# AgentCooper2002/AudioDiffuser

Hardware: AMD Instinct MI355X
Metric: audio samples/sec (16384-sample waveform, 50-step Heun) (higher is better)
Workload: dtype bf16; 1 GPU; BASELINE configs[1]: UNet1d 64 ch (c2), 16384-sample waveforms, KarrasSchedule N=50 heun, batch 64/GPU, random-init weights; global_batch=64, sampler=heun, num_steps=50, nfe=99, hipgraph=True, parallelism=batch-sharded x1, one all-gather

## Files before the change

### audiodiffuser_amd/csrc/adf_gemm.h

```cpp
#pragma once
#include "adf_common.h"

namespace adf {

constexpr int kARows = 144;
constexpr int kTapGroup = 3;

struct GemmSeg {
    const void* src0;
    const void* src1;
    int c0, c1;
    const float* ab;
    GnFinalizeArgs gn;
    float scale1;
    int act;
    int taps, stride, off0, step;
    const void* w;
    const void* wfrag;
    int nchunk;
};

struct GemmArgs {
    GemmSeg seg[2];
    int nseg;
    int B, lin, mrows, n, n_pad;
    int gn_ready;
    int flat;
    int seg_rows;
    const float* bias0;
    const float* bias1;
    int bias_mod;
    const void* res;
    int gelu;
    void* out;
    int out_rows, out_c;
    int scatter_f, scatter_pad;
    int phase_c;
    double* stats;
    int stats_groups;
};

template <int N>
__device__ __forceinline__ void gemm_bias_load(const GemmArgs& a, const int (&bi)[N], const bool (&ok)[N], float (&out)[N]) {
    const bool h0 = a.bias0 != nullptr, h1 = a.bias1 != nullptr;
    const float* const dmy = (const float*)a.seg[0].w;
    const float* const p0 = h0 ? a.bias0 : dmy;
    const float* const p1 = h1 ? a.bias1 : dmy;
    float v0[N], v1[N];
#pragma unroll
    for (int k = 0; k < N; ++k) {
        const int idx = ok[k] ? bi[k] : 0;
        v0[k] = p0[h0 ? idx : 0]; v1[k] = p1[h1 ? idx : 0];
// ... 1215 lines not shown
```

### audiodiffuser_amd/csrc/adf_gemm.hip

```cpp
#include "adf_gemm.h"
#include "adf_gemm_pp.h"
#include "adf_gemm_rb.h"
#include "adf_gemm_rbx3.h"
#include "adf_gemm_up.h"
#include "adf_kernels.h"
#include <cstdio>
#include <cstdlib>
#include <cstring>
#include <vector>


#ifdef ADF_RB_STAMP
namespace adf { __device__ unsigned long long adf_rb_stamps[8 * 16]; }
extern "C" int adf_debug_rb_stamps(unsigned long long* out) {
    return (int)hipMemcpyFromSymbol(out, HIP_SYMBOL(adf::adf_rb_stamps), sizeof(unsigned long long) * 8 * 16);
}
#endif

#ifdef ADF_RB_TL
namespace adf { __device__ unsigned adf_rb_tl[2 * 8 * 128]; }
extern "C" int adf_debug_rb_timeline(unsigned* out) {
    return (int)hipMemcpyFromSymbol(out, HIP_SYMBOL(adf::adf_rb_tl), sizeof(unsigned) * 2 * 8 * 128);
}
#endif
// ... 153 lines not shown
            e.src = (const char*)(from1 ? s1 : s0) + (size_t)(from1 ? c - c0 : c) * f.esz;
            e.pitch = (unsigned)(from1 ? c1 : c0) * (unsigned)f.esz;
            e.w = (const char*)w + (size_t)(c / f.blk_ch) * taps * a.n_pad * kRowBytes;
            e.tab = table ? c * 8 : -1;
            e.scale = from1 ? scale1 : 1.0f;
        }
    };
    add_seg(g0.src0, g0.src1, g0.c0, g0.c1, g0.w, 3, !raw0, 1.0f);
    r.h.nb3 = nb;
    if (a.nseg > 1) {
        const GemmSeg& g1 = a.seg[1];
        if (g1.taps != 1 || g1.off0 != 0 || g1.stride != 1 || g1.step != 1 || g1.ab || g1.gn.gamma || g1.act) return false;
        if (!seg_ok(g1.c0, g1.c1, nb)) return false;
        add_seg(g1.src0, g1.src1, g1.c0, g1.c1, g1.w, 1, false, g1.scale1);
    }
    r.h.res = a.nseg == 1 ? a.res : nullptr;
    r.h.nb1 = nb - r.h.nb3;
    r.h.B = a.B; r.h.L = a.mrows;
    r.h.n = a.n;
    r.h.gn = g0.gn;
    r.h.bias0 = a.bias0; r.h.bias1 = a.bias1;
    r.h.out = a.out;
    r.h.stats = nullptr; r.h.stats_groups = 0;
    if (a.phase_c && (!raw0 || (a.phase_c & (a.phase_c - 1)) || a.phase_c < 64 || a.n % a.phase_c)) return false;
    if (a.stats) {
        const int sc = a.phase_c ? a.phase_c : a.out_c;
        const int gs = a.stats_groups > 0 ? sc / a.stats_groups : 0;
        if (!(gs > 0 && gs * a.stats_groups == sc && (gs & (gs - 1)) == 0 && gs >= 8 && gs <= 64)) return false;
        r.h.stats = a.stats; r.h.stats_groups = a.stats_groups;
        r.h.stats_mod = a.phase_c;
    }
    return true;
}
static int rb_num_cus() {
    static int num_cu_dev[kMaxDevices] = {};
    int& n = num_cu_dev[current_device()];
    if (n == 0 && (hipDeviceGetAttribute(&n, hipDeviceAttributeMultiprocessorCount, current_device()) != hipSuccess || n < 1)) n = 256;
    return n;
}

bool try_launch_rb(const GemmArgs& a, const void* ident, long long min_tiles, hipStream_t stream, const char** err, bool dry = false) {
    *err = nullptr;
    (void)ident;
    auto pow2 = [](int v) { return v > 0 && (v & (v - 1)) == 0; };
    RbArgs r;
    bool raw0 = false;
    if (!rb_build_args(a, RbForm{2, 64, kRbMaxBlk, true}, r, raw0)) return false;
    static long long m128_nh = -1;
    if (m128_nh < 0) m128_nh = adf_tuning("ADF_RB_M128_NH", 1);
    auto shape = [&](int tm_, int& nh_) -> long long {
        if (a.mrows % tm_ || !pow2(a.mrows / tm_)) return 0;
        const long long tiles_m = (long long)a.B * (a.mrows / tm_);
        nh_ = (a.n == 256 && tiles_m >= min_tiles) ? 2 : 1;
        return tiles_m * (a.n / (kPpTN * nh_));
    };
    int tm = 256, nh = 1;
    long long tiles_total = shape(256, nh);
    bool wide128 = false;
    if (tiles_total < min_tiles) {
        tm = 128;
        tiles_total = shape(128, nh);
        if (m128_nh == 2 && a.n == 256 && nh == 1 && tiles_total >= min_tiles) { nh = 2; tiles_total /= 2; wide128 = true; }
    }
    if (tiles_total > (1 << 22) || tiles_total < (wide128 ? min_tiles / 2 : min_tiles)) return false;
    r.h.tiles_n = a.n / (kPpTN * nh);
    r.h.tm_shift = 0;
    while ((1 << r.h.tm_shift) < a.mrows / tm) ++r.h.tm_shift;
    r.h.tiles_total = (int)tiles_total;
    if (dry) return true;
    static bool attr_done[kMaxDevices] = {};
    const int dev = current_device();
    if (!attr_done[dev]) {
        bool ok = true;
        for (const void* k : {(const void*)conv_gemm_rb_kernel<1, false, 2>, (const void*)conv_gemm_rb_kernel<2, false, 2>, (const void*)conv_gemm_rb_kernel<1, true, 2>,
                              (const void*)conv_gemm_rb_kernel<2, true, 2>, (const void*)conv_gemm_rb_kernel<1, false, 1>, (const void*)conv_gemm_rb_kernel<2, false, 1>,
                              (const void*)conv_gemm_rb_kernel<1, true, 1>, (const void*)conv_gemm_rb_kernel<2, true, 1>})
            ok = ok && hipFuncSetAttribute(k, hipFuncAttributeMaxDynamicSharedMemorySize, kRbLds) == hipSuccess;
        if (!ok) {
            *err = "hipFuncSetAttribute(MaxDynamicSharedMemorySize, rb) failed";
            return true;
        }
        attr_done[dev] = true;
    }
    const int ncu = rb_num_cus();
    const long long grid = tiles_total < ncu ? tiles_total : ncu;
    auto go = [&](auto kern) { hipLaunchKernelGGL(kern, dim3((unsigned)grid), dim3(512), kRbLds, stream, r); };
    if (tm == 256) {
        if (nh == 2 && raw0) go(conv_gemm_rb_kernel<2, true, 2>);
        else if (nh == 2) go(conv_gemm_rb_kernel<2, false, 2>);
        else if (raw0) go(conv_gemm_rb_kernel<1, true, 2>);
        else go(conv_gemm_rb_kernel<1, false, 2>);
    } else {
        if (nh == 2 && raw0) go(conv_gemm_rb_kernel<2, true, 1>);
        else if (nh == 2) go(conv_gemm_rb_kernel<2, false, 1>);
        else if (raw0) go(conv_gemm_rb_kernel<1, true, 1>);
        else go(conv_gemm_rb_kernel<1, false, 1>);
    }
    if (hipGetLastError() != hipSuccess) *err = "conv_gemm_rb: launch failed";
    return true;
}

bool try_launch_rbx3(const GemmArgs& a, long long min_tiles, hipStream_t stream, const char** err, bool dry = false) {
// ... 76 lines not shown
    constexpr int lds = 4 * ks_wave_lds(MT, NT);
    constexpr int TM = 32 * MT, TN = 32 * NT;
    static bool attr_done[kMaxDevices] = {};
    bool& attr_set = attr_done[current_device()];
    auto kern = conv_gemm_ksplit_kernel<T, MT, NT>;
    if (!attr_set) {
        if (hipFuncSetAttribute((const void*)kern, hipFuncAttributeMaxDynamicSharedMemorySize, lds) != hipSuccess)
            return "hipFuncSetAttribute(MaxDynamicSharedMemorySize, ksplit) failed";
        attr_set = true;
    }
    const int tiles_n = (a.n_pad + TN - 1) / TN;
    const long long tiles_m = a.flat ? ((long long)a.B * a.mrows + TM - 1) / TM : (long long)((a.mrows + TM - 1) / TM) * a.B;
    const long long blocks = tiles_m * tiles_n;
    if (blocks <= 0 || blocks > 0x7fffffffLL) return "conv_gemm_ksplit: bad grid";
    hipLaunchKernelGGL(kern, dim3((unsigned)blocks), dim3(256), lds, stream, a);
    return hipGetLastError() == hipSuccess ? nullptr : "conv_gemm_ksplit: launch failed";
}

template <typename T>
const char* dispatch(const GemmArgs& a, int tm, int tn, hipStream_t s) {
    if (tm == 128 && tn == 128) return launch_variant<T, 2, 2, 2, 2>(a, s);
    if (tm == 128 && tn == 64) return launch_variant<T, 2, 1, 2, 2>(a, s);
    if (tm == 128 && tn == 32) return launch_variant<T, 1, 1, 4, 1>(a, s);
    if (tm == 64 && tn == 128) return launch_variant<T, 1, 2, 2, 2>(a, s);
    if (tm == 64 && tn == 64) return launch_variant<T, 1, 1, 2, 2>(a, s);
    if (tm == 64 && tn == 32) return launch_variant<T, 1, 1, 2, 1>(a, s);
    if (tm == 32 && tn == 128) return launch_variant<T, 1, 1, 1, 4>(a, s);
    if (tm == 32 && tn == 64) return launch_variant<T, 1, 1, 1, 2>(a, s);
    return launch_variant<T, 1, 1, 1, 1>(a, s);
}

}

static void trace_route(const char* route, const GemmArgs& a, int tm, int tn) {
    static int on = -1;
    if (on < 0) on = adf_route_switch("ADF_GEMM_TRACE", 0);
    if (!on) return;
    fprintf(stderr, "[adf gemm] %-6s B=%d lin=%d mrows=%d n=%d/%d nseg=%d seg0(c=%d+%d taps=%d stride=%d off0=%d step=%d ab=%d act=%d)", route, a.B, a.lin, a.mrows,
            a.n, a.n_pad, a.nseg, a.seg[0].c0, a.seg[0].c1, a.seg[0].taps, a.seg[0].stride, a.seg[0].off0, a.seg[0].step, a.seg[0].ab != nullptr, a.seg[0].act);
    if (a.nseg > 1) fprintf(stderr, " seg1(c=%d+%d taps=%d ab=%d)", a.seg[1].c0, a.seg[1].c1, a.seg[1].taps, a.seg[1].ab != nullptr);
    fprintf(stderr, " res=%d gelu=%d scatter=%d out=%dx%d stats=%d flat=%d tile=%dx%d\n", a.res != nullptr, a.gelu, a.scatter_f, a.out_rows, a.out_c, a.stats != nullptr,
            a.flat, tm, tn);
}

static long long rb_min_tiles() {
    static int use_rb = -1;
    if (use_rb < 0) use_rb = adf_route_switch("ADF_GEMM_RB", 1);
    return use_rb == 0 ? -1 : (use_rb >= 2 ? 32 : 256);
}
static long long rbx3_min_tiles() {
    static int use_rbx3 = -1;
    if (use_rbx3 < 0) use_rbx3 = adf_route_switch("ADF_GEMM_RBX3", 1);
    return use_rbx3 == 0 ? -1 : (use_rbx3 >= 2 ? 32 : 256);
}
bool conv_gemm_phase_eligible(const GemmArgs& a, int dtype) {
    const long long mt = dtype == 2 ? rbx3_min_tiles() : rb_min_tiles();
    if (dtype == 0 || mt < 0 || !a.phase_c || a.flat) return false;
    const char* err = nullptr;
    return dtype == 2 ? try_launch_rbx3(a, mt, nullptr, &err, true) : try_launch_rb(a, nullptr, mt, nullptr, &err, true);
}

const char* launch_conv_gemm(const GemmArgs& a_in, int dtype, hipStream_t stream, bool* stats_fused) {
    const bool dtype_bf16 = dtype == 1, x3 = dtype == 2;
    GemmArgs a = a_in;
    if (stats_fused) *stats_fused = false;
    if (a.phase_c) {
        const long long mt = x3 ? rbx3_min_tiles() : rb_min_tiles();
        if (dtype == 0 || mt < 0 || a.flat) return "conv_gemm: a 3-tap-form transposed conv that conv_gemm_rb_kernel does not take";
        const char* err = nullptr;
        auto go = [&]() { return x3 ? try_launch_rbx3(a, mt, stream, &err) : try_launch_rb(a, nullptr, mt, stream, &err); };
        bool taken = go();
        if (!taken && a.stats) { a.stats = nullptr; taken = go(); }
        if (!taken) return "conv_gemm: a 3-tap-form transposed conv that conv_gemm_rb_kernel does not take";
        if (stats_fused) *stats_fused = a.stats != nullptr;
        trace_route(x3 ? "rbx3" : "rb", a, 256, 128);
        return err;
    }
    if (a.nseg < 1 || a.nseg > 2) return "conv_gemm: nseg must be 1 or 2";
    if (a.n_pad % 32) return "conv_gemm: n_pad must be a multiple of 32";
    const int epc = dtype_bf16 ? 8 : 4;
    if (a.n % epc || a.out_c % epc) return "conv_gemm: output channels must be a multiple of a 16-byte chunk";
    const long long esz = dtype_bf16 ? 2 : 4;
    if ((long long)a.B * a.out_rows * a.out_c * esz >= (1LL << 32)) return "conv_gemm: output tensor must be < 4 GiB";
    const bool gn_pending = a.seg[0].gn.gamma != nullptr;
    static int gn_in_kernel = -1;
    if (gn_in_kernel < 0) gn_in_kernel = (int)adf_tuning("ADF_GEMM_GN", 1);
    auto settle_gn = [&](bool in_kernel) -> const char* {
        if (!gn_pending) return nullptr;
        const GnFinalizeArgs& gn = a.seg[0].gn;
        const int gn_gs = gn.G > 0 ? (gn.c0 + gn.c1) / gn.G : 0;
        in_kernel = in_kernel && gn_in_kernel && gn_gs > 0 && gn.c0 % gn_gs == 0;
        const char* err = nullptr;
        if (!in_kernel) {
            if (!a.gn_ready) err = launch_gn_finalize(a.seg[0].gn, stream);
            a.seg[0].gn.gamma = nullptr;
        }
        return err;
    };
    if (a.nseg > 1) a.seg[1].gn.gamma = nullptr;
    bool raw = true;
    for (int s = 0; s < a.nseg; ++s) {
        const GemmSeg& g = a.seg[s];
        if (g.c0 % epc || g.c1 % epc) return "conv_gemm: channel counts must be multiples of a 16-byte chunk";
        if (g.step != 1 && g.step != -1) return "conv_gemm: step must be +-1";
        if (g.taps < 1 || g.stride < 1) return "conv_gemm: bad taps/stride";
        if (g.ab) raw = false;
        if ((long long)a.B * a.lin * (g.c0 > g.c1 ? g.c0 : g.c1) * esz >= (1LL << 32)) return "conv_gemm: input tensor must be < 4 GiB";
    }
// ... 102 lines not shown
        }
    }
    {
        static int use_pp = -1;
        if (use_pp < 0) use_pp = adf_route_switch("ADF_GEMM_PP", 1);
        int ptm = 0;
        if (use_pp && dtype_bf16 && !flat && tm == 128) {
            const long long t256 = pp_eligible(a, 256) ? (long long)a.B * (a.mrows / 256) * (a.n_pad / kPpTN) : 0;
            const long long t128 = pp_eligible(a, 128) ? (long long)a.B * (a.mrows / 128) * (a.n_pad / kPpTN) : 0;
            const long long need = use_pp >= 2 ? 128 : 256;
            if (t256 >= need) ptm = 256;
            else if (t128 >= need && use_pp != 3) ptm = 128;
        }
        {
            static int use_rb = -1;
            if (use_rb < 0) use_rb = adf_route_switch("ADF_GEMM_RB", 1);
            const bool rb_raw = !gn_pending && !a.seg[0].ab && !a.seg[0].act && a.nseg == 1 && !a.res && a.seg[0].taps == 3;
            const long long rbx3_mt = rbx3_min_tiles();
            if (rbx3_mt >= 0 && x3 && !flat && ((gn_pending && gn_in_kernel && !a.gn_ready) || rb_raw)) {
                const char* err = nullptr;
                GemmArgs b = a;
                b.stats = a_in.stats;
                if (try_launch_rbx3(b, rbx3_mt, stream, &err)) {
                    if (stats_fused) *stats_fused = a_in.stats != nullptr;
                    trace_route("rbx3", a, 256, 128);
                    return err;
                }
            }
            if (use_rb && dtype_bf16 && !flat && ((gn_pending && gn_in_kernel && !a.gn_ready) || rb_raw)) {
                const char* err = nullptr;
                const void* ident = nullptr;
                GemmArgs b = a;
                b.stats = a_in.stats;
                if (try_launch_rb(b, ident, use_rb >= 2 ? 32 : 256, stream, &err)) {
                    if (stats_fused) *stats_fused = a_in.stats != nullptr;
                    trace_route("rb", a, 256, 128);
                    return err;
                }
            }
        }
        if (ptm) {
            static int pp_linear = -1;
            if (pp_linear < 0) pp_linear = (int)adf_tuning("ADF_GEMM_PP_LINEAR", 0);
            const bool linear = a.seg[0].taps == 1 && a.nseg == 1;
            const bool take = linear ? pp_linear != 0 : (use_pp == 2 || !a.res);
            if (take) {
                if (a_in.stats) {
                    const int gs = a.stats_groups > 0 ? a.out_c / a.stats_groups : 0;
                    const bool ok = gs > 0 && gs * a.stats_groups == a.out_c && (gs & (gs - 1)) == 0 && gs >= 8 && gs <= 64;
                    a.stats = ok ? a_in.stats : nullptr;
                    if (stats_fused) *stats_fused = ok;
                }
                if (a.res) {
                    const char* err = nullptr;
                    const void* ident = pp_identity(a.n, stream, &err);
                    if (!ident) return err;
                    GemmSeg& g = a.seg[1];
                    g = GemmSeg{};
                    g.src0 = a.res; g.src1 = nullptr; g.c0 = a.n; g.c1 = 0; g.ab = nullptr; g.scale1 = 1.0f; g.act = 0;
                    g.taps = 1; g.stride = 1; g.off0 = 0; g.step = 1; g.w = ident; g.nchunk = a.n / 64;
                    a.nseg = 2;
                    a.res = nullptr;
                }
                if (const char* e = settle_gn(a.seg[0].taps == 3)) return e;
                trace_route("pp", a, ptm, 128);
                return ptm == 256 ? launch_pp<2>(a, stream) : launch_pp<1>(a, stream);
            }
        }
    }
// ... 35 lines not shown
```

### audiodiffuser_amd/csrc/adf_gemm_rb.h

```cpp
#pragma once
#include "adf_gemm.h"
#include "adf_gemm_pp.h"
#include <type_traits>

namespace adf {

#ifdef ADF_RB_STAMP
extern __device__ unsigned long long adf_rb_stamps[8 * 16];
#endif

#ifdef ADF_RB_TL
extern __device__ unsigned adf_rb_tl[2 * 8 * 128];
constexpr int kRbLds = kPpLds + 3072;
#else
constexpr int kRbLds = kPpLds;
#endif
constexpr int kRbMaxBlk = 24;
#ifndef ADF_RB_KNOCK
#define ADF_RB_KNOCK 0
#endif
#ifndef ADF_RB_DOT2
#define ADF_RB_DOT2 1
#endif
#ifndef ADF_RB_NT
#define ADF_RB_NT 0
#endif
#ifndef ADF_RB_W3
#define ADF_RB_W3 1
#endif
#ifndef ADF_RB_PRIO
#define ADF_RB_PRIO 4
#endif
#ifndef ADF_RB_FILL2
#define ADF_RB_FILL2 1
#endif
#ifndef ADF_RB_PRESLAB
#define ADF_RB_PRESLAB 1
#endif


struct RbBlk {
    const char* src;
    const char* w;
    unsigned pitch;
    int tab;
    float scale;
    int pad_;
};

struct RbHead {
    int nb3, nb1;
    int B, L;
    int tm_shift;
    int tiles_n;
    int tiles_total;
    int n;
    GnFinalizeArgs gn;
    const float* bias0; const float* bias1;
    void* out;
    const void* res;
    double* stats; int stats_groups;
    int stats_mod;
};
struct RbArgs {
    RbHead h;
    RbBlk blk[kRbMaxBlk];
};

__device__ __forceinline__ void rb_dma2(const char* base, unsigned va, unsigned vb, unsigned la, unsigned lb) {
    asm volatile("s_mov_b32 m0, %3\n\ts_nop 0\n\tglobal_load_lds_dwordx4 %1, %0\n\t"
                 "s_mov_b32 m0, %4\n\ts_nop 0\n\tglobal_load_lds_dwordx4 %2, %0"
                 :: "s"(base), "v"(va), "v"(vb), "s"(la), "s"(lb) : "memory");
}
__device__ __forceinline__ void rb_dma1(const char* base, unsigned va, unsigned la) {
    asm volatile("s_mov_b32 m0, %2\n\ts_nop 0\n\tglobal_load_lds_dwordx4 %1, %0" :: "s"(base), "v"(va), "s"(la) : "memory");
}

template <int I, int N, typename F>
__device__ __forceinline__ void rb_static_for(F&& f) {
    if constexpr (I < N) {
        f(std::integral_constant<int, I>{});
        rb_static_for<I + 1, N>(f);
    }
}

template <int NH, bool RAW, int MH = 2>
__global__ void __launch_bounds__(512) conv_gemm_rb_kernel(const RbArgs a) {
    typedef bf16_t T;
    constexpr int TM = 128 * MH, HP = TM / 8;
    constexpr int TNB = kPpTN * NH;
    constexpr bool W3 = ADF_RB_W3 == 2 || (ADF_RB_W3 == 1 && (MH == 1 || NH == 2)) || (ADF_RB_W3 == 3 && MH == 1) || (ADF_RB_W3 == 4 && (MH == 1 || NH == 1));
    extern __shared__ __attribute__((aligned(16))) char smem[];
    const RbHead H = a.h;
    const RbBlk e_first[3] = {a.blk[0], a.blk[1], a.blk[2]};
    asm volatile("" :: "s"(H.nb3), "s"(H.tiles_total), "s"(H.gn.stats0), "s"(H.gn.gamma), "s"(H.gn.film), "s"(H.bias0), "s"(H.out), "s"(H.stats),
                 "s"(e_first[0].src), "s"(e_first[1].src), "s"(e_first[2].src), "s"(e_first[0].tab), "s"(e_first[1].tab), "s"(e_first[2].tab));
    char* const ldsScr = smem + kPpOffScr;
    char* const ldsTab = smem + kPpOffTab;
    float* const ldsBias = (float*)(smem + kPpOffBias);

    const int tid = threadIdx.x, lane = tid & 63;
    const int wave = __builtin_amdgcn_readfirstlane(tid >> 6);
    const int r = lane & 31, h = lane >> 5;
    const int wm = wave >> 1, wn = wave & 1;
    const int lrow = lane >> 3;
    const int chunk = (lane & 7) ^ ((((wave & 1) << 2) + (lane >> 4)) & 7);
    const int srow = wave * 8 + lrow;
    const unsigned lane_lds = (unsigned)lane * 16u;

    if (ADF_RB_PRIO == 4) __builtin_amdgcn_s_setprio(3);
    if (ADF_RB_PRIO == 1 && wave >= 4) __builtin_amdgcn_s_setprio(1);
    if (ADF_RB_PRIO == 3 && wave >= 4) __builtin_amdgcn_s_setprio(2);
    const int nblk_grid = (int)gridDim.x, bidx = (int)blockIdx.x;
    const int t_lo = (int)((unsigned)bidx * (unsigned)H.tiles_total / (unsigned)nblk_grid);
    const int t_hi = (int)((unsigned)(bidx + 1) * (unsigned)H.tiles_total / (unsigned)nblk_grid);
    const int ntiles = t_hi - t_lo;
    if (ntiles <= 0) return;
    const int nb3 = H.nb3, nb1 = H.nb1, nb = nb3 + nb1;
    const int ctot0 = H.gn.c0 + H.gn.c1;
    const int tn_shift = H.tiles_n > 1 ? 1 : 0;
    const int tm_mask = (1 << H.tm_shift) - 1;

    struct Tile { int b0, m0, n0; };
    auto tile_of = [&](int tseq) __attribute__((always_inline)) -> Tile {
        const int t = t_lo + tseq;
        const int tml = t >> tn_shift;
        Tile g;
        g.n0 = (t & (H.tiles_n - 1)) * TNB;
        g.b0 = tml >> H.tm_shift;
        g.m0 = (tml & tm_mask) * TM;
        return g;
    };
    const int b_first = tile_of(0).b0;

    struct Blk {
        const char* abase;
        const char* w;
        unsigned pitch;
        int tab;
        float scale;
        int edge;
        int taps;
    };
    int d_t = 0, d_k = 0;
    Tile d_tile = tile_of(0);
    auto make_desc_of = [&](const RbBlk& e) __attribute__((always_inline)) -> Blk {
        Blk d;
        const int three = d_k < nb3;
        const int p_lo = d_tile.m0 - three;
        d.pitch = e.pitch;
        d.abase = e.src + (long long)(d_tile.b0 * H.L + p_lo) * (long long)e.pitch;
        d.w = e.w + (unsigned)d_tile.n0 * (unsigned)kRowBytes;
        d.tab = e.tab >= 0 ? ((d_tile.b0 - b_first) & 1) * kPpTab + e.tab : -1;
        d.scale = e.scale;
        d.taps = three ? 3 : 1;
        d.edge = three ? ((d_tile.m0 == 0 ? 1 : 0) | (d_tile.m0 + TM >= H.L ? 2 : 0)) : 0;
        return d;
    };
    auto make_desc = [&]() __attribute__((always_inline)) -> Blk { return make_desc_of(a.blk[d_k]); };
    auto advance = [&]() __attribute__((always_inline)) {
        if (++d_k == nb) {
            d_k = 0;
            if (++d_t < ntiles) d_tile = tile_of(d_t);
        }
    };
    const unsigned slab = (unsigned)H.n * (unsigned)kRowBytes;

    const unsigned colbytes = (unsigned)chunk * 16u;
    auto issue_a01 = [&](const Blk& d, unsigned st) __attribute__((always_inline)) {
        if (ADF_RB_KNOCK & 2) return;
        const unsigned v = (unsigned)srow * d.pitch + colbytes;
        const unsigned v0 = ((d.edge & 1) && srow == 0) ? v + d.pitch : v;
        const unsigned l = st + (unsigned)wave * 1024u;
        rb_dma2(d.abase, v0, v + 64u * d.pitch, l, l + 8192u);
    };
    auto issue_a23 = [&](const Blk& d, unsigned st) __attribute__((always_inline)) {
        if ((ADF_RB_KNOCK & 2) || MH == 1) return;
        const unsigned v = (unsigned)(srow + 128) * d.pitch + colbytes;
        const unsigned l = st + (unsigned)wave * 1024u + 16384u;
        rb_dma2(d.abase, v, v + 64u * d.pitch, l, l + 8192u);
    };
    auto issue_halo = [&](const Blk& d, unsigned st) __attribute__((always_inline)) {
        if (ADF_RB_KNOCK & 2) return;
        if (wave == 0 && d.taps == 3) {
            const unsigned vh = (unsigned)TM * d.pitch + ((d.edge & 2) ? 0u : (unsigned)lrow * d.pitch) + colbytes;
            if (lane < 16) rb_dma1(d.abase, vh, st + (unsigned)HP * 1024u);
        }
    };
    const unsigned wlane = (unsigned)srow * (unsigned)kRowBytes + colbytes;
// ... 116 lines not shown
        char* const ldsH = smem + st + HP * 1024 + lane_lds;
        const bool halo = wave == 0 && d.taps == 3 && lane < 16;
        const bool act = true;
        float fa[8], fb[8];
        load_ab(d, 0, 8, fa, fb);
#pragma unroll
        for (int u = 0; u < 2 * MH; ++u) {
            const u32x4_t q = *(const u32x4_t*)(ldsA + u * 8192);
            const u32x2_t lo = silu4(u32x2_t{q.x, q.y}, fa, fb, act), hi = silu4(u32x2_t{q.z, q.w}, fa + 4, fb + 4, act);
            *(u32x4_t*)(ldsA + u * 8192) = u32x4_t{lo.x, lo.y, hi.x, hi.y};
        }
        if (halo) {
            const u32x4_t q = *(const u32x4_t*)ldsH;
            const u32x2_t lo = silu4(u32x2_t{q.x, q.y}, fa, fb, act), hi = silu4(u32x2_t{q.z, q.w}, fa + 4, fb + 4, act);
            *(u32x4_t*)ldsH = u32x4_t{lo.x, lo.y, hi.x, hi.y};
        }
        zero_fill(d, st);
    };

    f32x16_t acc[NH][MH][2];
    unsigned abase0[3];
#pragma unroll
    for (int t = 0; t < 3; ++t) {
        const int row = wm * 32 * MH + r + t, f = (row >> 1) & 7;
        abase0[t] = (unsigned)(row * kPpRow + ((h ^ (f & 1)) << 4) + ((f >> 1) << 5));
    }
    const int fw = (r >> 1) & 7;
    const unsigned wbase0 = (unsigned)((wn * 64 + r) * kPpRow + ((h ^ (fw & 1)) << 4) + ((fw >> 1) << 5));
    unsigned wadr[4];
#pragma unroll
    for (int ks = 0; ks < 4; ++ks) wadr[ks] = (unsigned)kPpOffW + (wbase0 ^ (unsigned)(ks << 5));

    unsigned ws0 = 0u, ws1 = (unsigned)kPpWStage, ws2 = 2u * (unsigned)kPpWStage;
    auto substep = [&](auto tapc, auto wstc, auto nhc, unsigned sa_, auto work, auto mid) __attribute__((always_inline)) {
        constexpr int TAP = decltype(tapc)::value;
        constexpr int WST = decltype(wstc)::value;
        constexpr int H = decltype(nhc)::value;
        const char* const pw = smem + (W3 ? ws0 : (unsigned)(WST * kPpWStage));
        unsigned aadr[4];
#pragma unroll
        for (int ks = 0; ks < 4; ++ks) aadr[ks] = sa_ + (abase0[TAP] ^ (unsigned)(ks << 5));
        bf16x8_t fa[2][MH], fb[2][2];
#pragma unroll
        for (int i = 0; i < MH; ++i) fa[0][i] = *(const bf16x8_t*)(smem + aadr[0] + i * 32 * kPpRow);
#pragma unroll
        for (int j = 0; j < 2; ++j) fb[0][j] = *(const bf16x8_t*)(pw + wadr[0] + j * 32 * kPpRow);
#pragma unroll
        for (int ks = 0; ks < 4; ++ks) {
            const int cur = ks & 1, nxt = cur ^ 1;
            if (ks + 1 < 4) {
#pragma unroll
                for (int i = 0; i < MH; ++i) fa[nxt][i] = *(const bf16x8_t*)(smem + aadr[ks + 1] + i * 32 * kPpRow);
#pragma unroll
                for (int j = 0; j < 2; ++j) fb[nxt][j] = *(const bf16x8_t*)(pw + wadr[ks + 1] + j * 32 * kPpRow);
            }
#pragma unroll
            for (int i = 0; i < MH; ++i)
#pragma unroll
                for (int j = 0; j < 2; ++j) {
                    if (!(ADF_RB_KNOCK & 8)) acc[H][i][j] = __builtin_amdgcn_mfma_f32_32x32x16_bf16(fa[cur][i], fb[cur][j], acc[H][i][j], 0, 0, 0);
                    else { asm volatile("" :: "v"(fa[cur][i]), "v"(fb[cur][j])); }
                    __builtin_amdgcn_sched_barrier(0);
                    if (!(ADF_RB_KNOCK & 1)) work(ks * 2 * MH + i * 2 + j);
                    __builtin_amdgcn_sched_barrier(0);
                }
            mid(ks);
            if (ADF_RB_PRIO == 4) {
                if (ks == 0) __builtin_amdgcn_s_setprio(2);
                else if (ks == 1) __builtin_amdgcn_s_setprio(1);
                else if (ks == 2) __builtin_amdgcn_s_setprio(0);
            }
            if (ADF_RB_PRIO == 2 && ks == 1 && wave >= 4) __builtin_amdgcn_s_setprio(2);
            if (ADF_RB_PRIO == 3 && ks == 1 && wave >= 4) __builtin_amdgcn_s_setprio(0);
            __builtin_amdgcn_sched_barrier(0);
        }
        if (ADF_RB_PRIO == 2 && wave >= 4) __builtin_amdgcn_s_setprio(0);
        if (ADF_RB_PRIO == 3 && wave >= 4) __builtin_amdgcn_s_setprio(2);
        if (ADF_RB_PRIO == 4) __builtin_amdgcn_s_setprio(3);
    };

    struct Part {
        u32x2_t raw[3];
        float ta[8], tb[8];
        float x[4], u[4];
        u32x2_t pk;
        float ec, ed;
        unsigned hraw;
        float ha, hb, hx, hu;
    };
    const unsigned halo_e = (unsigned)wave * 16u + ((unsigned)lane & 15u);
    auto half_of = [](int P, int k) constexpr -> int { return P < 2 ? P + 2 * k : 6 + k; };
    auto part_begin = [&](auto partc, const Blk& dn, unsigned sn, Part& p) __attribute__((always_inline)) {
        constexpr int P = decltype(partc)::value;
        char* const ldsN = smem + sn + wave * 1024 + lane_lds;
        if (P == 0) {
            load_ab(dn, 0, 4, p.ta, p.tb);
            p.ec = dn.tab >= 0 ? -1.4426950408889634f : 0.0f;
            p.ed = dn.tab >= 0 ? 0.0f : -200.0f;
        } else if (P == 1) load_ab(dn, 4, 4, p.ta + 4, p.tb + 4);
        constexpr int NOWN = MH == 2 ? (P < 2 ? 3 : 2) : (P < 2 ? 2 : 0);
#pragma unroll
        for (int k = 0; k < NOWN; ++k) {
            const int hh = half_of(P, k);
            p.raw[k] = *(const u32x2_t*)(ldsN + (hh >> 1) * 8192 + (hh & 1) * 8);
        }
        if (P == 2) {
            p.hraw = *(const unsigned short*)(smem + sn + HP * 1024 + halo_e * 2u);
            if (dn.tab >= 0) {
                const f32x2_t t = *(const f32x2_t*)(ldsTab + dn.tab + (halo_e & 63u) * 8u);
                p.ha = t.x; p.hb = t.y;
            } else { p.ha = dn.scale; p.hb = 0.f; }
// ... 179 lines not shown
    unsigned* const tl_lds = (unsigned*)(smem + kPpOffBias + 1024) + wave * 128;
    auto tl = [&](int id) __attribute__((always_inline)) {
        if (tl_which >= 0 && id < 128) {
            const unsigned long long t = __builtin_amdgcn_s_memtime();
            if (lane == 0) tl_lds[id] = (unsigned)t;
        }
    };
    auto tl_real = [&](int id) __attribute__((always_inline)) {
        if (tl_which >= 0) {
            const unsigned long long t = __builtin_amdgcn_s_memrealtime();
            if (lane == 0) { tl_lds[id] = (unsigned)t; tl_lds[id + 1] = (unsigned)(t >> 32); }
        }
    };
    if (tl_which >= 0) for (int i = lane; i < 128; i += 64) tl_lds[i] = 0u;
    int tl_sub = 0;
    tl_real(120);
    tl(0);
#else
    auto tl = [&](int) __attribute__((always_inline)) {};
#endif
    kstamp(11);
    tl(110);
    const bool hb0 = H.bias0 != nullptr, hb1 = H.bias1 != nullptr;
    const float* const dummy_f = (const float*)a.blk[0].w;
    const int bidx_l = tid < H.n ? tid : 0;
    const float b0v = (hb0 ? H.bias0 : dummy_f)[bidx_l], b1v = (hb1 ? H.bias1 : dummy_f)[bidx_l];
    GnLoaded gl = {};
    if constexpr (!RAW) gl = gn_load(b_first, tid < ctot0 ? tid : ctot0 - 1);
    tl(111);
    Blk dc = make_desc_of(e_first[0]);
    advance();
    issue_a01(dc, 0u); issue_a23(dc, 0u); issue_halo(dc, 0u);
    issue_w(dc.w, 0);
    if (W3 && !ADF_RB_FILL2) issue_w(dc.w + (unsigned)(1 / NH) * slab + (unsigned)(1 % NH) * (unsigned)kPpWStage, 1);
    Blk d1 = make_desc_of(e_first[1]);
    advance();
    if (!ADF_RB_FILL2) { issue_a01(d1, (unsigned)kPpAStage); issue_a23(d1, (unsigned)kPpAStage); issue_halo(d1, (unsigned)kPpAStage); }
    Blk d2 = make_desc_of(d_k == 0 ? e_first[0] : e_first[2]);
    advance();
    tl(112);
#ifdef ADF_RB_TL
    asm volatile("" :: "v"(gl.gamma), "v"(gl.beta), "v"(gl.f1s), "v"(gl.f1h), "v"(gl.f2s), "v"(gl.f2h), "v"(gl.s0), "v"(gl.q0), "v"(gl.s1), "v"(gl.q1), "v"(b0v), "v"(b1v));
    tl(113);
#endif
    if (tid < H.n) ldsBias[tid] = (hb0 ? b0v : 0.f) + (hb1 ? b1v : 0.f);
    if (!RAW && tid < ctot0) gn_store(tid, gl, 0);
    kstamp(12);
    tl(1);
    asm volatile("s_waitcnt vmcnt(0)" ::: "memory");
    if (ADF_RB_FILL2) {
        if (W3) issue_w(dc.w + (unsigned)(1 / NH) * slab + (unsigned)(1 % NH) * (unsigned)kPpWStage, 1);
        issue_a01(d1, (unsigned)kPpAStage); issue_a23(d1, (unsigned)kPpAStage); issue_halo(d1, (unsigned)kPpAStage);
    }
    __syncthreads();
    kstamp(13);
    tl(2);
    Tile cur_tile = tile_of(0);
#pragma unroll
    for (int hf = 0; hf < NH; ++hf) {
        float bias_r[2];
#pragma unroll
        for (int j = 0; j < 2; ++j) bias_r[j] = ldsBias[cur_tile.n0 + hf * kPpTN + wn * 64 + j * 32 + r];
#pragma unroll
        for (int i = 0; i < MH; ++i)
#pragma unroll
            for (int j = 0; j < 2; ++j)
#pragma unroll
                for (int e = 0; e < 16; ++e) acc[hf][i][j][e] = bias_r[j];
    }
    if (RAW) zero_fill(dc, 0u); else transform_all(dc, 0u);
    if (ADF_RB_FILL2) asm volatile("s_waitcnt vmcnt(0)" ::: "memory");
    asm volatile("s_waitcnt lgkmcnt(0)\n\ts_barrier" ::: "memory");
    kstamp(14);
    tl(3);

    unsigned sa = 0u, sa1 = (unsigned)kPpAStage, sa2 = 2u * (unsigned)kPpAStage;
    const std::integral_constant<int, 0> c0{};
    const std::integral_constant<int, 1> c1{};
    const std::integral_constant<int, 2> c2{};
    auto lds_barrier = [&]() __attribute__((always_inline)) { asm volatile("s_waitcnt lgkmcnt(0)\n\ts_barrier" ::: "memory"); };
    auto rotate = [&]() __attribute__((always_inline)) {
        const unsigned t = sa; sa = sa1; sa1 = sa2; sa2 = t;
        dc = d1; d1 = d2; d2 = make_desc();
        advance();
// ... 118 lines not shown
            const std::integral_constant<int, (WP + u) & 1> wstc{};
            const std::integral_constant<int, u> hfc{};
            int wq = 0, aq = 0;
            substep(c0, wstc, hfc, sa, [](int) __attribute__((always_inline)) {},
                    [&](int ks) __attribute__((always_inline)) {
                        if (ks == 0) {
                            if (W3) wq = issue_ahead(u + 2, NH, has1, has2);
                            else if (u + 1 < NH) issue_w(next_slab(u + 1, 1), (WP + u + 1) & 1);
                            else if (has1) issue_w(d1.w, (WP + u + 1) & 1);
                        } else if (u == NH - 1 && has2) {
                            if (ks == 1) { issue_a01(d2, sa2); aq += 2; }
                            else if (ks == 2) { issue_a23(d2, sa2); if (MH == 2) aq += 2; }
                            else { issue_halo(d2, sa2); if (wave == 0 && d2.taps == 3) aq += 1; }
                        }
                    });
            if (W3) {
                wait_n((u == NH - 1 ? 0 : aq_prev) + wq + aq);
                aq_prev = aq;
                w_rotate();
                if (u == NH - 1 && has1) transform_all(d1, sa1);
            } else if (u == NH - 1) {
                if (has2) {
                    if (MH == 2) { if (wave == 0 && d2.taps == 3) asm volatile("s_waitcnt vmcnt(5)" ::: "memory"); else asm volatile("s_waitcnt vmcnt(4)" ::: "memory"); }
                    else { if (wave == 0 && d2.taps == 3) asm volatile("s_waitcnt vmcnt(3)" ::: "memory"); else asm volatile("s_waitcnt vmcnt(2)" ::: "memory"); }
                }
                else asm volatile("s_waitcnt vmcnt(0)" ::: "memory");
                if (has1) transform_all(d1, sa1);
            } else {
                asm volatile("s_waitcnt vmcnt(0)" ::: "memory");
            }
            lds_barrier();
        });
    };
    constexpr int kPar3 = (3 * NH) & 1, kPar1 = NH & 1;

    for (; tseq < ntiles; ++tseq) {
        cur_tile = tile_of(tseq);
#ifdef ADF_RB_TL
        tl_sub = 0;
        tl(4 + tseq * 26);
#endif
        if (tseq > 0) {
#ifdef ADF_RB_STAMP
            if (tseq == 1) kstamp(15);
#endif
            if (ADF_RB_PRESLAB) {
                if (prev_one) { asm volatile("s_waitcnt vmcnt(0)" ::: "memory"); aq_prev = 0; prev_one = false; }
                if (!W3) { issue_w(next_slab(1, 3), 1); slab1_pre = true; }
                epi_vm = NH * 4 * MH * (H.res != nullptr ? 2 : 1) + (H.stats != nullptr ? 2 * NH : 0);
            }
            epilogue(tile_of(tseq - 1), cur_tile.n0, sa2);
        }
#ifdef ADF_RB_TL
        tl(4 + tseq * 26 + 1);
#endif
        for (kb = 0; kb < nb3; kb += 2) {
            block3(c0); rotate(); --remaining; prev_one = false;
            block3(std::integral_constant<int, kPar3>{}); rotate(); --remaining;
        }
        for (int k1 = 0; k1 < nb1; k1 += 2) {
            block1(c0); rotate(); --remaining;
            block1(std::integral_constant<int, kPar1>{}); rotate(); --remaining; prev_one = true;
        }
    }
    {
        const Tile last = tile_of(ntiles - 1);
        tl(108);
        epilogue(last, 0, sa2);
        tl(109);
    }
#ifdef ADF_RB_TL
    tl_real(122);
    if (tl_which >= 0) {
        asm volatile("s_waitcnt lgkmcnt(0)" ::: "memory");
        for (int i = lane; i < 128; i += 64) adf_rb_tl[(tl_which * 8 + wave) * 128 + i] = tl_lds[i];
    }
#endif
}

}
```

### audiodiffuser_amd/csrc/adf_net_unet1d.hip

```cpp
#include "adf_api_internal.h"

using namespace adf;
using namespace adf_api;

namespace adf_api {

struct ResW {
    int cin = 0, cout = 0, film_off = 0;
    float *g1w = nullptr, *g1b = nullptr, *g2w = nullptr, *g2b = nullptr;
    ConvW c1, c2, cr;
    bool has_res = false;
};
struct TrW {
    int c = 0, mid = 0;
    float *lnw = nullptr, *lnb = nullptr, *g0 = nullptr, *g3 = nullptr;
    ConvW qkv, proj, ff1, ff2;
};
struct DownW { ConvW down; std::vector<ResW> blocks; bool attn = false; TrW tr; int factor = 1, cin = 0, cout = 0; };
struct UpW { std::vector<ResW> blocks; bool attn = false; TrW tr; ConvW up; ConvW up3; int factor = 1, cin = 0, cout = 0; bool nearest = false; };

struct Unet1dNet : Net {
    adf_net_config cfg;
    float *to_in_w = nullptr, *to_out_w = nullptr, *fourier = nullptr, *t_w1 = nullptr, *t_b1 = nullptr, *t_w2 = nullptr, *t_b2 = nullptr;
    std::vector<DownW> downs;
// ... 371 lines not shown
        R.reg_f32(fn.pre + ".to_cond_embedding.1.bias", fn.rows, h->film_b + fn.off);
    }
    return R.ok ? 0 : fail(h, "device allocation failed while building the weight registry");
}

int Unet1dNet::forward(adf_handle* h, Plan* p, const FwdIO& io, hipStream_t s) {
    const adf_net_config& c = cfg;
    Walker1d W{{h, p, s}, c};
    W.film2 = io.film2; W.film2_bstride = io.film2_bstride;
    W.film = io.film_pre ? io.film_pre : p->film;
    if (W.begin()) return 1;
    const int B = p->B, L = p->L, n = c.num_layers;
    const int pad = c.window_length / 2 - c.stride / 2;
    const int tdim = 4 * c.channels;
    if (W.live() && !io.film_pre) {
        W.check(time_embed(io.t, io.t_stride, io.nb, p->temb, s));
        W.check(launch_film(p->temb, tdim, h->film_w, tdim + h->cdim, 0, h->film_b, p->film, io.nb, h->film_total, s));
    }
    Act x = W.new_act(c.num_filters, L / c.stride);
    if (W.live())
        W.check(launch_to_in(io.x, to_in_w, x.p, h->bf16, B, c.in_channels, L, c.num_filters, c.window_length, c.stride, pad,
                             io.coef, io.coef_bstride, s));
    W.tap("to_in", x);
    std::vector<std::vector<Act>> skips_list;
    for (int i = 0; i < n; ++i) {
        const DownW& d = downs[i];
        const int f = d.factor, km = c.kernel_multiplier_downsample;
        Act y = W.new_act(d.cout, x.L / f);
        if (x.L % f) return fail(h, "downsample: length not divisible by the factor");
        Act xv = x;
        xv.C = x.C * f; xv.L = x.L / f; xv.stats = nullptr;
        GemmArgs g = W.gemm_base(y, xv.L, y.L, d.down);
        g.seg[0] = Walker1d::seg_of(xv, nullptr, nullptr, 1.f, 0, km + 1, 1, -(km / 2), 1, d.down);
        W.run_gemm(g, y, true);
        W.tap("down" + std::to_string(i) + ".conv", y);
        x = y;
        std::vector<Act> skips;
        for (size_t j = 0; j < d.blocks.size(); ++j) {
            x = W.resblock("down" + std::to_string(i) + ".block" + std::to_string(j), x, nullptr, d.blocks[j], io.nb);
            skips.push_back(x);
        }
        if (d.attn) {
            x = W.transformer("down" + std::to_string(i) + ".attn", x, d.tr);
            skips.push_back(x);
        }
        skips_list.push_back(skips);
    }
    x = W.resblock("mid.pre", x, nullptr, mid_pre, io.nb);
    if (c.use_attention_bottleneck) x = W.transformer("mid.attn", x, mid_tr);
    x = W.resblock("mid.post", x, nullptr, mid_post, io.nb);
    for (int u = 0; u < n; ++u) {
        const UpW& up = ups[u];
        std::vector<Act>& skips = skips_list.back();
        for (size_t j = 0; j < up.blocks.size(); ++j) {
            if (skips.empty()) { W.check("upsample: skip stack underflow"); break; }
            Act sk = skips.back();
            skips.pop_back();
            x = W.resblock("up" + std::to_string(u) + ".block" + std::to_string(j), x, &sk, up.blocks[j], io.nb);
        }
        skips_list.pop_back();
        if (up.attn) x = W.transformer("up" + std::to_string(u) + ".attn", x, up.tr);
        const int f = up.factor;
        Act y = W.new_act(up.cout, x.L * f);
        bool done = false;
        if (up.nearest) {
            Act u0 = W.new_act(up.cin, x.L * f + 2);
// ... 62 lines not shown
```

Before: 4.393 million audio-samples/s.

## Skip structurally-zero weight slabs in raw rb conv GEMM kernel

Computes on the host a per-K-block mask of weight tap slabs that are structurally zero. These come from folded downsample convs, where taps beyond the kernel length are padding, and from phase-split transposed convs. The raw-input rb kernel then walks a reduced substep sequence that skips those MFMA substeps and their weight loads. This cuts MMA work and LDS traffic for those layers. The cost is a more complex per-block dynamic schedule, and forcing W3 triple-buffering for the RAW variant could change register and LDS pressure.

After: 4.430 million audio-samples/s, median of 6. No clear change (+0.9%).

```diff
diff --git a/audiodiffuser_amd/csrc/adf_gemm.h b/audiodiffuser_amd/csrc/adf_gemm.h
--- a/audiodiffuser_amd/csrc/adf_gemm.h
+++ b/audiodiffuser_amd/csrc/adf_gemm.h
@@ -18,6 +18,7 @@
     const void* w;
     const void* wfrag;
     int nchunk;
+    int fold_f, fold_k;
 };
 
 struct GemmArgs {
diff --git a/audiodiffuser_amd/csrc/adf_gemm.hip b/audiodiffuser_amd/csrc/adf_gemm.hip
--- a/audiodiffuser_amd/csrc/adf_gemm.hip
+++ b/audiodiffuser_amd/csrc/adf_gemm.hip
@@ -209,6 +209,43 @@
     }
     return true;
 }
+static int zskip_level() {
+    static int v = -1;
+    if (v < 0) v = adf_route_switch("ADF_GEMM_ZSKIP", 1);
+    return v;
+}
+static bool rb_slab_is_zero(const GemmArgs& a, int c, int tap, int col0, int ncol) {
+    const GemmSeg& g = a.seg[0];
+    if (g.taps != 3 || g.c1 != 0) return false;
+    if (g.fold_f > 0 && g.fold_k > 0 && !a.phase_c) {
+        if (g.c0 % g.fold_f) return false;
+        const int cin = g.c0 / g.fold_f;
+        return cin > 0 && tap * g.fold_f + (c * 64) / cin >= g.fold_k;
+    }
+    if (a.phase_c > 0 && a.n % a.phase_c == 0) {
+        const int f = a.n / a.phase_c;
+        if (f < 2 || f % 2) return false;
+        const int p_lo = col0 / a.phase_c, p_hi = (col0 + ncol - 1) / a.phase_c;
+        return tap == 0 ? p_lo >= f / 2 : (tap == 2 ? p_hi < f / 2 : false);
+    }
+    return false;
+}
+static void rb_fill_zmask(const GemmArgs& a, RbArgs& r, bool raw0, int nh, int* zs) {
+    zs[0] = 0; zs[1] = r.h.nb3 * 3 * nh + r.h.nb1 * nh;
+    if (!raw0 || zskip_level() < 1) return;
+    for (int c = 0; c < r.h.nb3; ++c) {
+        int m[2] = {0, 0};
+        for (int hidx = 0; hidx < a.n / kPpTN; ++hidx)
+            for (int tap = 0; tap < 3; ++tap)
+                if (rb_slab_is_zero(a, c, tap, hidx * kPpTN, kPpTN)) m[hidx] |= 1 << tap;
+        int z = 0;
+        if (nh == 2) z = m[0] | (m[1] << 3);
+        else if (a.n == kPpTN || m[0] == m[1]) z = m[0];
+        if (z != (nh == 2 ? kRbZTwo2 : kRbZTwo1) && !(nh == 2 && z == kRbZPhase2)) z = 0;
+        r.blk[c].zmask = z;
+        zs[0] += __builtin_popcount((unsigned)z);
+    }
+}
 static int rb_num_cus() {
     static int num_cu_dev[kMaxDevices] = {};
     int& n = num_cu_dev[current_device()];
@@ -216,7 +253,7 @@
     return n;
 }
 
-bool try_launch_rb(const GemmArgs& a, const void* ident, long long min_tiles, hipStream_t stream, const char** err, bool dry = false) {
+bool try_launch_rb(const GemmArgs& a, const void* ident, long long min_tiles, hipStream_t stream, const char** err, bool dry = false, int* zs = nullptr) {
     *err = nullptr;
     (void)ident;
     auto pow2 = [](int v) { return v > 0 && (v & (v - 1)) == 0; };
@@ -245,6 +282,8 @@
     while ((1 << r.h.tm_shift) < a.mrows / tm) ++r.h.tm_shift;
     r.h.tiles_total = (int)tiles_total;
     if (dry) return true;
+    int zs_local[2];
+    rb_fill_zmask(a, r, raw0, nh, zs ? zs : zs_local);
     static bool attr_done[kMaxDevices] = {};
     const int dev = current_device();
     if (!attr_done[dev]) {
@@ -387,7 +426,7 @@
 
 }
 
-static void trace_route(const char* route, const GemmArgs& a, int tm, int tn) {
+static void trace_route(const char* route, const GemmArgs& a, int tm, int tn, const int* zs = nullptr) {
     static int on = -1;
     if (on < 0) on = adf_route_switch("ADF_GEMM_TRACE", 0);
     if (!on) return;
@@ -396,6 +435,9 @@
     if (a.nseg > 1) fprintf(stderr, " seg1(c=%d+%d taps=%d ab=%d)", a.seg[1].c0, a.seg[1].c1, a.seg[1].taps, a.seg[1].ab != nullptr);
     fprintf(stderr, " res=%d gelu=%d scatter=%d out=%dx%d stats=%d flat=%d tile=%dx%d\n", a.res != nullptr, a.gelu, a.scatter_f, a.out_rows, a.out_c, a.stats != nullptr,
             a.flat, tm, tn);
+    if (zs)
+        fprintf(stderr, "[adf zskip] %-6s B=%d mrows=%d n=%d c=%d act=%d fold=%d/%d phase_c=%d zskip=%d/%d\n", route, a.B, a.mrows, a.n, a.seg[0].c0 + a.seg[0].c1,
+                a.seg[0].act, a.seg[0].fold_f, a.seg[0].fold_k, a.phase_c, zs[0], zs[1]);
 }
 
 static long long rb_min_tiles() {
@@ -423,12 +465,13 @@
         const long long mt = x3 ? rbx3_min_tiles() : rb_min_tiles();
         if (dtype == 0 || mt < 0 || a.flat) return "conv_gemm: a 3-tap-form transposed conv that conv_gemm_rb_kernel does not take";
         const char* err = nullptr;
-        auto go = [&]() { return x3 ? try_launch_rbx3(a, mt, stream, &err) : try_launch_rb(a, nullptr, mt, stream, &err); };
+        int zs[2] = {0, 0};
+        auto go = [&]() { return x3 ? try_launch_rbx3(a, mt, stream, &err) : try_launch_rb(a, nullptr, mt, stream, &err, false, zs); };
         bool taken = go();
         if (!taken && a.stats) { a.stats = nullptr; taken = go(); }
         if (!taken) return "conv_gemm: a 3-tap-form transposed conv that conv_gemm_rb_kernel does not take";
         if (stats_fused) *stats_fused = a.stats != nullptr;
-        trace_route(x3 ? "rbx3" : "rb", a, 256, 128);
+        trace_route(x3 ? "rbx3" : "rb", a, 256, 128, x3 ? nullptr : zs);
         return err;
     }
     if (a.nseg < 1 || a.nseg > 2) return "conv_gemm: nseg must be 1 or 2";
@@ -597,9 +640,10 @@
                 const void* ident = nullptr;
                 GemmArgs b = a;
                 b.stats = a_in.stats;
-                if (try_launch_rb(b, ident, use_rb >= 2 ? 32 : 256, stream, &err)) {
+                int zs[2] = {0, 0};
+                if (try_launch_rb(b, ident, use_rb >= 2 ? 32 : 256, stream, &err, false, zs)) {
                     if (stats_fused) *stats_fused = a_in.stats != nullptr;
-                    trace_route("rb", a, 256, 128);
+                    trace_route("rb", a, 256, 128, zs);
                     return err;
                 }
             }
diff --git a/audiodiffuser_amd/csrc/adf_gemm_rb.h b/audiodiffuser_amd/csrc/adf_gemm_rb.h
--- a/audiodiffuser_amd/csrc/adf_gemm_rb.h
+++ b/audiodiffuser_amd/csrc/adf_gemm_rb.h
@@ -45,8 +45,9 @@
     unsigned pitch;
     int tab;
     float scale;
-    int pad_;
+    int zmask;
 };
+constexpr int kRbZTwo1 = 4, kRbZTwo2 = 4 | (4 << 3), kRbZPhase2 = 4 | (1 << 3);
 
 struct RbHead {
     int nb3, nb1;
@@ -89,7 +90,7 @@
     typedef bf16_t T;
     constexpr int TM = 128 * MH, HP = TM / 8;
     constexpr int TNB = kPpTN * NH;
-    constexpr bool W3 = ADF_RB_W3 == 2 || (ADF_RB_W3 == 1 && (MH == 1 || NH == 2)) || (ADF_RB_W3 == 3 && MH == 1) || (ADF_RB_W3 == 4 && (MH == 1 || NH == 1));
+    constexpr bool W3 = RAW || ADF_RB_W3 == 2 || (ADF_RB_W3 == 1 && (MH == 1 || NH == 2)) || (ADF_RB_W3 == 3 && MH == 1) || (ADF_RB_W3 == 4 && (MH == 1 || NH == 1));
     extern __shared__ __attribute__((aligned(16))) char smem[];
     const RbHead H = a.h;
     const RbBlk e_first[3] = {a.blk[0], a.blk[1], a.blk[2]};
@@ -141,6 +142,8 @@
         float scale;
         int edge;
         int taps;
+        int nsub;
+        unsigned seq;
     };
     int d_t = 0, d_k = 0;
     Tile d_tile = tile_of(0);
@@ -155,6 +158,11 @@
         d.scale = e.scale;
         d.taps = three ? 3 : 1;
         d.edge = three ? ((d_tile.m0 == 0 ? 1 : 0) | (d_tile.m0 + TM >= H.L ? 2 : 0)) : 0;
+        if constexpr (RAW) {
+            const bool two = e.zmask == (NH == 2 ? kRbZTwo2 : kRbZTwo1), phase = NH == 2 && e.zmask == kRbZPhase2;
+            d.nsub = two ? 2 * NH : (phase ? 4 : 3 * NH);
+            d.seq = two ? (NH == 2 ? 0x3210u : 0x10u) : (phase ? 0x5230u : (NH == 2 ? 0x543210u : 0x210u));
+        }
         return d;
     };
     auto make_desc = [&]() __attribute__((always_inline)) -> Blk { return make_desc_of(a.blk[d_k]); };
@@ -337,14 +345,13 @@
     for (int ks = 0; ks < 4; ++ks) wadr[ks] = (unsigned)kPpOffW + (wbase0 ^ (unsigned)(ks << 5));
 
     unsigned ws0 = 0u, ws1 = (unsigned)kPpWStage, ws2 = 2u * (unsigned)kPpWStage;
-    auto substep = [&](auto tapc, auto wstc, auto nhc, unsigned sa_, auto work, auto mid) __attribute__((always_inline)) {
-        constexpr int TAP = decltype(tapc)::value;
+    auto substep_at = [&](unsigned ab_, auto wstc, auto nhc, unsigned sa_, auto work, auto mid) __attribute__((always_inline)) {
         constexpr int WST = decltype(wstc)::value;
         constexpr int H = decltype(nhc)::value;
         const char* const pw = smem + (W3 ? ws0 : (unsigned)(WST * kPpWStage));
         unsigned aadr[4];
 #pragma unroll
-        for (int ks = 0; ks < 4; ++ks) aadr[ks] = sa_ + (abase0[TAP] ^ (unsigned)(ks << 5));
+        for (int ks = 0; ks < 4; ++ks) aadr[ks] = sa_ + (ab_ ^ (unsigned)(ks << 5));
         bf16x8_t fa[2][MH], fb[2][2];
 #pragma unroll
         for (int i = 0; i < MH; ++i) fa[0][i] = *(const bf16x8_t*)(smem + aadr[0] + i * 32 * kPpRow);
@@ -382,6 +389,9 @@
         if (ADF_RB_PRIO == 2 && wave >= 4) __builtin_amdgcn_s_setprio(0);
         if (ADF_RB_PRIO == 3 && wave >= 4) __builtin_amdgcn_s_setprio(2);
         if (ADF_RB_PRIO == 4) __builtin_amdgcn_s_setprio(3);
+    };
+    auto substep = [&](auto tapc, auto wstc, auto nhc, unsigned sa_, auto work, auto mid) __attribute__((always_inline)) {
+        substep_at(abase0[decltype(tapc)::value], wstc, nhc, sa_, work, mid);
     };
 
     struct Part {
@@ -627,7 +637,12 @@
     advance();
     issue_a01(dc, 0u); issue_a23(dc, 0u); issue_halo(dc, 0u);
     issue_w(dc.w, 0);
-    if (W3 && !ADF_RB_FILL2) issue_w(dc.w + (unsigned)(1 / NH) * slab + (unsigned)(1 % NH) * (unsigned)kPpWStage, 1);
+    auto second_slab = [&]() __attribute__((always_inline)) -> const char* {
+        int u = 1;
+        if constexpr (RAW) u = (int)((dc.seq >> 4) & 15u);
+        return dc.w + (unsigned)(u / NH) * slab + (unsigned)(u % NH) * (unsigned)kPpWStage;
+    };
+    if (W3 && !ADF_RB_FILL2) issue_w(second_slab(), 1);
     Blk d1 = make_desc_of(e_first[1]);
     advance();
     if (!ADF_RB_FILL2) { issue_a01(d1, (unsigned)kPpAStage); issue_a23(d1, (unsigned)kPpAStage); issue_halo(d1, (unsigned)kPpAStage); }
@@ -644,7 +659,7 @@
     tl(1);
     asm volatile("s_waitcnt vmcnt(0)" ::: "memory");
     if (ADF_RB_FILL2) {
-        if (W3) issue_w(dc.w + (unsigned)(1 / NH) * slab + (unsigned)(1 % NH) * (unsigned)kPpWStage, 1);
+        if (W3) issue_w(second_slab(), 1);
         issue_a01(d1, (unsigned)kPpAStage); issue_a23(d1, (unsigned)kPpAStage); issue_halo(d1, (unsigned)kPpAStage);
     }
     __syncthreads();
@@ -829,6 +844,56 @@
             lds_barrier();
         });
     };
+    auto zslab_of = [&](const Blk& d, int v) __attribute__((always_inline)) -> const char* {
+        const unsigned u = (d.seq >> (4 * v)) & 15u;
+        return d.w + (u / (unsigned)NH) * slab + (u % (unsigned)NH) * (unsigned)kPpWStage;
+    };
+    auto issue_ahead_z = [&](int v, int ucur, bool has1, bool has2) __attribute__((always_inline)) -> int {
+        if (v < ucur) { issue_w_at(zslab_of(dc, v), ws2); return 2; }
+        v -= ucur;
+        if (!has1) return 0;
+        const int u1 = d1.nsub;
+        if (v < u1) { issue_w_at(zslab_of(d1, v), ws2); return 2; }
+        if (!has2) return 0;
+        issue_w_at(zslab_of(d2, v - u1), ws2);
+        return 2;
+    };
+    auto block_raw = [&]() __attribute__((always_inline)) {
+        const bool has1 = remaining > 1, has2 = remaining > 2;
+        const int U = dc.nsub;
+        for (int i = 0; i < U; i += NH) {
+            rb_static_for<0, NH>([&](auto hc) __attribute__((always_inline)) {
+                constexpr int hf = decltype(hc)::value;
+                const int v = i + hf;
+                const unsigned tap = ((dc.seq >> (4 * v)) & 15u) / (unsigned)NH;
+                const unsigned ab = tap == 0u ? abase0[0] : (tap == 1u ? abase0[1] : abase0[2]);
+                int wq = 0, aq = 0;
+                substep_at(ab, c0, hc, sa, [](int) __attribute__((always_inline)) {},
+                           [&](int ks) __attribute__((always_inline)) {
+                               if (ks == 0) wq = issue_ahead_z(v + 2, U, has1, has2);
+                               else if (ks == 1 && has2) {
+                                   if (v == 0) { issue_halo(d2, sa2); issue_a01(d2, sa2); aq = (wave == 0 && d2.taps == 3) ? 3 : 2; }
+                                   else if (v == 1 && MH == 2) { issue_a23(d2, sa2); aq = 2; }
+                               }
+                           });
+                if (v == U - 1) zero_fill(d1, sa1);
+#ifdef ADF_RB_TL
+                tl(4 + tseq * 26 + 2 + 2 * tl_sub);
+#endif
+                if (v == 0 && epi_vm > 0) {
+                    wait_upto(epi_vm + aq_prev + wq + aq);
+                    epi_vm = 0;
+                } else wait_n((v == U - 1 ? 0 : aq_prev) + wq + aq);
+                aq_prev = aq;
+                w_rotate();
+                lds_barrier();
+#ifdef ADF_RB_TL
+                tl(4 + tseq * 26 + 3 + 2 * tl_sub);
+                ++tl_sub;
+#endif
+            });
+        }
+    };
     constexpr int kPar3 = (3 * NH) & 1, kPar1 = NH & 1;
 
     for (; tseq < ntiles; ++tseq) {
@@ -851,6 +916,13 @@
 #ifdef ADF_RB_TL
         tl(4 + tseq * 26 + 1);
 #endif
+        if constexpr (RAW) {
+            for (kb = 0; kb < nb3; ++kb) {
+                block_raw();
+                rotate(); --remaining;
+            }
+            continue;
+        }
         for (kb = 0; kb < nb3; kb += 2) {
             block3(c0); rotate(); --remaining; prev_one = false;
             block3(std::integral_constant<int, kPar3>{}); rotate(); --remaining;
diff --git a/audiodiffuser_amd/csrc/adf_net_unet1d.hip b/audiodiffuser_amd/csrc/adf_net_unet1d.hip
--- a/audiodiffuser_amd/csrc/adf_net_unet1d.hip
+++ b/audiodiffuser_amd/csrc/adf_net_unet1d.hip
@@ -427,6 +427,7 @@
         xv.C = x.C * f; xv.L = x.L / f; xv.stats = nullptr;
         GemmArgs g = W.gemm_base(y, xv.L, y.L, d.down);
         g.seg[0] = Walker1d::seg_of(xv, nullptr, nullptr, 1.f, 0, km + 1, 1, -(km / 2), 1, d.down);
+        g.seg[0].fold_f = d.down.f; g.seg[0].fold_k = d.down.K;
         W.run_gemm(g, y, true);
         W.tap("down" + std::to_string(i) + ".conv", y);
         x = y;
```
